# zhangyi-3/UCDIR

Hardware: AMD Instinct MI355X
Metric: restored images/sec at 50-step p_sample_loop, 256x256 SID (higher is better)
Workload: dtype bf16

## Files before the change

ucdir_amd/csrc/engine.hip:

```cpp
#include <hip/hip_runtime.h>

#include <cmath>
#include <cstdio>
#include <cstring>
#include <map>
#include <mutex>
#include <set>
#include <array>
#include <atomic>
#include <memory>
#include <string>
#include <vector>

#include "../../include/ucdir_hip.h"
#include "cgemm.hip.h"
#include "conv_halo.hip.h"
#include "akgm_halo.hip.h"
#include "akgm_pre.hip.h"
#include "akgm_ws.hip.h"
#include "akgm_ws32.hip.h"
#include "akgm_ws64.hip.h"
#include "conv_ws.hip.h"
#include "conv_sk.hip.h"
#include "conv_ws128.hip.h"
#include "flash_attn2.hip.h"
#include "qkv_ws.hip.h"
#include "common.h"
#include "misc.hip.h"
#include "fewstep.hip.h"
#include "image_metrics.hip.h"
#include "jpeg_roundtrip.hip.h"
#include "pack.h"

static thread_local std::string g_err;
static int fail(const std::string& m) { g_err = m; return 1; }
#define HIPC(x)                                                                                   \
    do {                                                                                          \
        hipError_t e_ = (x);                                                                      \
        if (e_ != hipSuccess) {                                                                   \
            throw std::runtime_error(std::string(#x) + ": " + hipGetErrorString(e_));             \
        }                                                                                         \
    } while (0)
#define API_BEGIN try {
#define API_END                                                                                   \
    }                                                                                             \
    catch (const std::exception& e) { return fail(e.what()); }                                    \
    catch (...) { return fail("unknown error"); }                                                 \
// ... 27 lines not shown
        return p;
    }
    static constexpr size_t STAT_CAP = 1 << 21;
    stat_t* stat_slab = nullptr; size_t stat_used = 0;
    stat_t* alloc_stats(int B) {
        if (!stat_slab) stat_slab = (stat_t*)alloc(STAT_CAP * sizeof(stat_t), true);
        const size_t n = (size_t)2 * UCDIR_STAT_SLOTS * B;
        if (stat_used + n > STAT_CAP) throw std::runtime_error("DevPool: statistics slab exhausted");
        stat_t* p = stat_slab + stat_used; stat_used += n;
        return p;
    }
    void zero_stats(hipStream_t st) { if (stat_used) HIPC(hipMemsetAsync(stat_slab, 0, stat_used * sizeof(stat_t), st)); }
    void release() { for (void* p : ptrs) (void)hipFree(p); ptrs.clear(); bytes = 0; stat_slab = nullptr; stat_used = 0; }
    ~DevPool() { release(); }
};

struct ConvW {
    bf16_t* A = nullptr; float* bias = nullptr; float* Tb = nullptr; float* Tg = nullptr;
    int rows_pad = 0, Kpad = 0, ntaps = 0, cin = 0, cout = 0, TM = 128; bool fold = false;
    bf16_t* Aup = nullptr; int Kup = 0;
    bf16_t* A10 = nullptr; float* bias_res = nullptr;
    bf16_t* Aws = nullptr;
    bf16_t* Aws128 = nullptr;
    bf16_t* Aqkv = nullptr;
    bf16_t* Atile = nullptr;
    bf16_t* Ask[2] = {nullptr, nullptr}; bf16_t* Ask_up[2] = {nullptr, nullptr};
    long long sk_up_stride[2] = {0, 0};
    bf16_t* Ask1x1 = nullptr;
};
struct AkgmW {
    bf16_t* A = nullptr; float* bias = nullptr; float* Tb = nullptr; float* Tg = nullptr;
    float* Tbb = nullptr;
    bf16_t* Apre = nullptr;
    bf16_t* Aws32 = nullptr;
    bf16_t* Aws64 = nullptr;
    int C = 0, cg = 0, Kpad = 0;
};

static int pick_tm(int cout) { return cout >= 128 ? 128 : 64; }

static ConvW upload_conv(DevPool& pool, const float* w, const float* bias, const float* gamma, const float* beta,
                         int cout, int cin, int ks) {
    ConvW W;
    W.TM = pick_tm(cout);
    PackedConv P = pack_conv(w, bias, gamma, beta, cout, cin, ks, W.TM);
    W.A = pool.upload(P.A); W.bias = pool.upload(P.bias);
// ... 103 lines not shown
    StampDump(hipStream_t, StampLayout) {}
    unsigned long long* dbg() const { return nullptr; }
    template <typename H> void print(H) const {}
#endif
};

struct Env {
    static bool has(const char* n) { return getenv(n) != nullptr; }
    static bool is0(const char* n) { const char* v = getenv(n); return v && atoi(v) == 0; }
    const bool no_pre = has("UCDIR_NO_PRE");
    const bool no_attlds = has("UCDIR_NO_ATTLDS");
    const bool no_ws = has("UCDIR_NO_WS");
    const bool no_ws16 = has("UCDIR_NO_WS16");
    const bool no_ws32 = has("UCDIR_NO_WS32");
    const bool no_ws64 = has("UCDIR_NO_WS64");
    const bool no_owntc = has("UCDIR_NO_OWNTC");
    const bool no_conv_sk = has("UCDIR_NO_CONV_SK");
    const bool sk_mix = !is0("UCDIR_SK_MIX");
    const bool no_tail_res = has("UCDIR_NO_TAIL_RES");
    const bool no_fused_res = has("UCDIR_NO_FUSED_RES");
    const bool no_atile = has("UCDIR_NO_ATILE");
    const bool no_conv_ws = has("UCDIR_NO_CONV_WS");
    const bool no_conv_ws128 = has("UCDIR_NO_CONV_WS128");
    const bool no_qkv_ws = has("UCDIR_NO_QKV_WS");
    const bool no_flash = has("UCDIR_NO_FLASH");
    const bool no_fused_final = has("UCDIR_NO_FUSED_FINAL");
    const bool splitk = !is0("UCDIR_SPLITK");
    const int splitk_wgs = has("UCDIR_SPLITK_WGS") ? atoi(getenv("UCDIR_SPLITK_WGS")) : 256;
    const bool keep_acts = has("UCDIR_KEEP_ACTS");
    const bool prof_detail = has("UCDIR_PROF_DETAIL");
};
static const Env& env() { static const Env e; return e; }

template <int TM, int EPI, int MODE>
static void launch_one(const GemmP& p, dim3 grid, size_t lds, hipStream_t st) {
    hipLaunchKernelGGL((cgemm_kernel<TM, EPI, MODE>), grid, dim3(CG_THREADS), lds, st, p);
}

template <typename K> static void set_lds_attr(K* k, int bytes, bool abs0 = false) {
    HIPC(hipFuncSetAttribute((const void*)k, hipFuncAttributeMaxDynamicSharedMemorySize, bytes));
    if (abs0) {
        hipFuncAttributes fa;
        HIPC(hipFuncGetAttributes(&fa, (const void*)k));
        require(fa.sharedSizeBytes == 0, "a kernel with absolute LDS addressing has static __shared__ memory: its dynamic smem[] no longer starts at offset 0");
    }
}
// ... 5 lines not shown
#define SPLITK_MAX_WGS 512
#define SK_MAX_GRID 256
#define SCRATCH_BYTES ((size_t)2 * SK_MAX_GRID * 65536 * sizeof(float))
static std::map<int, float*> g_splitk_buf;
static std::mutex g_static_mu;
static void ensure_kernel_attrs() {
    std::lock_guard<std::mutex> lk(g_static_mu);
    static std::set<int> done;
    int dev = 0;
    HIPC(hipGetDevice(&dev));
    if (done.count(dev)) return;
    set_cgemm_attrs<64>(); set_cgemm_attrs<128>();
    set_lds_attr(conv3x3_halo_kernel<128, false>, hc_lds_bytes<128>());
    set_lds_attr(conv3x3_halo_kernel<64, false>, hc_lds_bytes<64>());
    set_lds_attr(conv3x3_halo_kernel<64, true>, hc_lds_bytes<64>());
    set_lds_attr(akgm_halo_stage_kernel, AH_LDS); set_lds_attr(akgm_halo_kernel<true>, AH_LDS);
    set_lds_attr(akgm_pre_kernel<8>, AkPre<8>::LDS);
    set_lds_attr(akgm_ws_kernel<8>, AkWs::LDS); set_lds_attr(akgm_ws_kernel<16>, AkWs::LDS);
    set_lds_attr(akgm_ws32_kernel<32>, AkWs32::LDS); set_lds_attr(akgm_ws32_kernel<16>, AkWs32::LDS); set_lds_attr(akgm_ws32_kernel<8>, AkWs32::LDS);
    set_lds_attr(akgm_ws64_kernel<2, 8, true>, 160 * 1024); set_lds_attr(akgm_ws64_kernel<4, 8, true>, 160 * 1024);
    set_lds_attr(qkv_ws_kernel<256>, QkvWs::LDS); set_lds_attr(qkv_ws_kernel<512>, QkvWs::LDS);
    set_lds_attr(conv_ws_kernel, CvWs::LDS);
    set_lds_attr(conv_ws128_kernel, CvWs128::LDS);
    set_lds_attr(conv_sk_kernel<2, 8, 9>, 160 * 1024); set_lds_attr(conv_sk_kernel<2, 8, 4>, 160 * 1024);
    set_lds_attr(conv_sk_kernel<1, 8, 9>, 160 * 1024); set_lds_attr(conv_sk_kernel<1, 8, 4>, 160 * 1024);
    set_lds_attr(conv_sk_kernel<1, 4, 9>, 80 * 1024, true); set_lds_attr(conv_sk_kernel<1, 4, 4>, 80 * 1024, true);

    set_lds_attr(final_conv_kernel, 160 * 1024);
    set_lds_attr(flash_attn2_kernel<1, false>, fa_lds_bytes(128), true); set_lds_attr(flash_attn2_kernel<1, true>, fa_lds_bytes(128), true);
    set_lds_attr(flash_attn2_kernel<2, false>, fa_lds_bytes(256), true); set_lds_attr(flash_attn2_kernel<2, true>, fa_lds_bytes(256), true);
    set_lds_attr(flash_attn2_kernel<3, false>, fa_lds_bytes(384), true); set_lds_attr(flash_attn2_kernel<3, true>, fa_lds_bytes(384), true);
    set_lds_attr(flash_attn2_kernel<4, false>, fa_lds_bytes(512), true); set_lds_attr(flash_attn2_kernel<4, true>, fa_lds_bytes(512), true);
    done.insert(dev);
}

static void gemm_work(const GemmP& p, int epi, double& flops, double& bytes) {
    const double cols = ((p.cols_mode == COLS_PLAIN) ? (double)p.W : (double)p.H * p.W) * (p.up_phase ? 4.0 : 1.0);
    if (epi == EPI_AKGM) {
        const double C = 8.0 * p.cg;
        flops = 2.0 * 9 * C * C * cols * p.nbatch;
        bytes = (2.0 * C * cols * 2 + C * cols * 2 + cols * 32) * p.nbatch + 9.0 * C * C * 2;
    } else {
        const double K = (double)p.ntaps * p.cg;
        flops = 2.0 * K * p.nfeat * cols * p.nbatch;
        double in_cols = cols;
        if (p.cols_mode == COLS_DOWN) in_cols = cols * 4; else if (p.cols_mode == COLS_UP) in_cols = cols / 4;
// ... 66 lines not shown
    memo[{H, W}] = {th, tw};
}

template <int TM, bool DUAL = false>
static void launch_halo(GemmP p, hipStream_t st) {
    const int ks = p.ksplit > 1 ? p.ksplit : 1;
    const int nblk = p.nbatch * p.tiles_x * p.tiles_y * p.rowtiles * (p.up_phase ? 4 : 1) * ks + p.alt_blocks;
    ProfEntry e = gemm_entry((TM == 128 ? KEY_HALO128 : KEY_HALO64) + (p.up_phase ? KEY_HALO_UP : 0) + (DUAL ? KEY_HALO_DUAL : 0), p, EPI_STD, p.cg);
    if (p.alt_blocks) add_res_rider(e, p);
    StampDump sd(st, STAMPS_256); p.dbg = sd.dbg();
    bracket(e, st, [&] {
        hipLaunchKernelGGL((conv3x3_halo_kernel<TM, DUAL>), dim3(nblk), dim3(HC_THREADS), hc_lds_bytes<TM>(), st, p);
        if (ks == 1) return;
        const long long items = (long long)p.H * p.W * (p.up_phase ? 4 : 1) * (p.nfeat / 8);
        int gx = (int)((items + 255) / 256); if (gx > 1024) gx = 1024;
        hipLaunchKernelGGL(conv_splitk_finish_kernel, dim3(gx, p.nbatch), dim3(256), 0, st, p, TM);
    });
    sd.print([](int, int n) { fprintf(stderr, "TIMING n=%d:", n); });
}

static std::atomic<bool> g_use_halo{true};

static std::atomic<int> g_wsb{-1};
static std::atomic<int> g_persist_grid{0};
static int num_cus() {
    if (g_persist_grid > 0) return g_persist_grid;
    static std::map<int, int> memo;
    static std::mutex mu;
    std::lock_guard<std::mutex> lk(mu);
    int dev = 0;
    HIPC(hipGetDevice(&dev));
    auto it = memo.find(dev);
    if (it != memo.end()) return it->second;
    int n = 0;
    HIPC(hipDeviceGetAttribute(&n, hipDeviceAttributeMultiprocessorCount, dev));
    if (n <= 0) n = 256;
    memo[dev] = n;
    return n;
}

static thread_local float* t_splitk = nullptr;
static float* splitk_scratch() {
    if (t_splitk) return t_splitk;
    std::lock_guard<std::mutex> lk(g_static_mu);
    int dev = 0;
    HIPC(hipGetDevice(&dev));
// ... 148 lines not shown
                2.0 * 9 * cin * (double)w.cout * cols,
                ((double)cin * H * W * 2 + (double)w.cout * cols / B * 2) * B + 9.0 * cin * w.cout * 2, H, W, cin, w.cout};
    if (p.alt_units) { e.flops += 2.0 * cin * (double)w.cout * cols; e.bytes += 2.0 * cin * w.cout + 2.0 * w.cout * cols; }
    StampDump sd(st, STAMPS_CONV_SK); p.dbg = sd.dbg();
    bracket(e, st, [&] {
        if (upph) hipLaunchKernelGGL((conv_sk_kernel<MW, NW, 4>), dim3(G), dim3(L::THREADS), lds, st, p);
        else hipLaunchKernelGGL((conv_sk_kernel<MW, NW, 9>), dim3(G), dim3(L::THREADS), lds, st, p);
        if (nsk > 0) hipLaunchKernelGGL((conv_sk_finish_kernel<MW, NW>), dim3(4 * NW, nsk), dim3(64), 0, st, p, Gmain);
    });
    sd.print([&](int win, int n) { fprintf(stderr, "CONV_SK TIMING %s units=%d grid=%d n=%d:", win ? "last-round" : "first-round", p.units, G, n); });
    return true;
}
static bool try_conv_sk(const ConvW& w, ConvCall& c, bool upph, hipStream_t st) {
    const int mode = g_convsk.load();
    if (mode == 0 || (mode < 0 && env().no_conv_sk)) return false;
    if (c.x0.C % 32 || (c.x1 && c.x1->C % 32) || c.y.C % 8) return false;
    const int kind = mode > 0 ? mode : 2;
    const int fm = mode > 0 ? 1 : -1;
    if (kind == 2) return try_conv_sk_mw<1, 4>(w, c, upph, st, fm);
    if (w.cout % 256 == 0) return try_conv_sk_mw<2, 8>(w, c, upph, st, fm);
    return try_conv_sk_mw<1, 8>(w, c, upph, st, fm);
}

enum class ConvKind { WS128, WS, HALO128, HALO64, HALO64_DUAL, CGEMM };

static bool run_conv(const ConvW& w, int mode, ConvCall c, hipStream_t st) {
    const Act &x0 = c.x0, &y = c.y; const Act* x1 = c.x1;
    GemmP p; zero_gemm(p);
    const int cin = x0.C + (x1 ? x1->C : 0);
    require(cin == w.cin, "run_conv: channel mismatch");
    require(y.C == w.cout, "run_conv: cout mismatch");
    p.A = w.A; p.a_ld = w.Kpad; p.a_rows = w.rows_pad;
    p.B0 = x0.p; p.b0_bstride = x0.bstride(); p.ld0 = x0.C; p.c0 = x0.C;
    if (x1) { p.B1 = x1->p; p.b1_bstride = x1->bstride(); p.ld1 = x1->C; }
    p.cols_mode = mode;
    p.H = y.H; p.W = y.W; p.Wp = y.W + 2;
    p.Hi = x0.H; p.Wi = x0.W; p.Wpi = x0.W + 2;
    p.p0 = p.Wp + 1; p.pn = (y.H - 1) * p.Wp + y.W;
    p.ntaps = w.ntaps; p.cg = cin; p.cpt = cin / 8; p.cpt_shift = 0;
    p.nk = w.Kpad / CG_BK;
    p.tiles = (p.pn + CG_TP - 1) / CG_TP;
    p.rowtiles = w.rows_pad / w.TM;
    p.nbatch = y.B;
    p.fold = w.fold ? 1 : 0; p.act = c.act;
    if (w.fold) {
        p.stats0 = x0.stats; p.stats1 = x1 ? x1->stats : nullptr;
        p.inv_count = 1.0 / ((double)cin * x0.H * x0.W);
// ... 30 lines not shown
        p.A = w.A10; p.a_ld = 10 * cin; p.res_fused = 1; p.bias2 = w.bias_res;
        p.out2 = c.res_out->p; p.out2_bstride = c.res_out->bstride(); p.out2_ld = c.res_out->C;
        did_res = true;
    }
    const bool dual = did_res;
    if (!env().no_atile && halo && !upph && !did_res && tm_run == w.TM && w.Atile && w.ntaps == 9) p.A_tiled = w.Atile;
    if (halo && !did_res && !p.out_nchw && w.cout % 8 == 0) {
        const int taps = upph ? 4 : 9, tps = 256 / tm_run;
        const int ks = choose_ksplit(p.nbatch * p.tiles * p.rowtiles, cin / HC_BK, (taps + tps - 1) / tps,
                                     (double)y.B * y.H * y.W * w.cout);
        if (ks > 1) { p.ksplit = ks; p.partial = splitk_scratch(); }
    }
    if (halo && !upph && !did_res && c.res_out && c.wres && !env().no_tail_res && !p.out_nchw && c.wres->ntaps == 1 &&
        c.wres->rows_pad >= p.rowtiles * tm_run) {
        p.alt_blocks = p.nbatch * p.tiles * p.rowtiles;
        p.alt_A = c.wres->A; p.alt_a_ld = c.wres->Kpad; p.bias2 = c.wres->bias;
        p.out2 = c.res_out->p; p.out2_bstride = c.res_out->bstride(); p.out2_ld = c.res_out->C;
        did_res = true;
    }
    ConvKind kind = !halo ? ConvKind::CGEMM : tm_run == 128 ? ConvKind::HALO128 : dual ? ConvKind::HALO64_DUAL : ConvKind::HALO64;
    if (!env().no_conv_ws128 && dual && w.Aws128 && cin == 128 && x0.C == 64 && x1 && x1->C == 64 && !c.res && !p.out_nchw && y.H % 8 == 0 && y.W % 16 == 0 &&
        y.C == 64 && (g_persist_grid > 0 || (long long)y.B * (y.H / 8) * (y.W / 16) >= 4LL * num_cus()))
        kind = ConvKind::WS128;
    else if (!env().no_conv_ws && halo && !upph && !did_res && w.Aws && !x1 && !c.res && !p.out_nchw && p.ksplit <= 1 && !p.alt_blocks &&
             y.H % 16 == 0 && y.W % 16 == 0 && x0.C == 64 && y.C == 64 &&
             (g_persist_grid > 0 || (long long)y.B * (y.H / 16) * (y.W / 16) >= 4LL * num_cus()))
        kind = ConvKind::WS;

    switch (kind) {
        case ConvKind::WS128: {
            p.A = w.Aws128; p.alt_A = w.Aws128 + (size_t)2 * 72 * 2 * 32 * 8;
            p.th = 8; p.tw = 16; p.tiles_x = y.W / 16; p.tiles_y = y.H / 8;
            const int ntiles = y.B * p.tiles_x * p.tiles_y, ncu = num_cus();
            const int grid = ntiles < ncu ? ntiles : ncu;
            ProfEntry e = gemm_entry(KEY_CONV_WS128, p, EPI_STD, p.cg);
            add_res_rider(e, p);
            StampDump sd(st, STAMPS_256); p.dbg = sd.dbg();
            bracket(e, st, [&] { hipLaunchKernelGGL(conv_ws128_kernel, dim3(grid), dim3(CvWs128::THREADS), CvWs128::LDS, st, p); });
            sd.print([](int, int n) { fprintf(stderr, "CONV_WS128 TIMING n=%d:", n); });
            break;
        }
        case ConvKind::WS: {
            p.A = w.Aws; p.th = 16; p.tw = 16; p.tiles_x = y.W / 16; p.tiles_y = y.H / 16;
            const int ntiles = y.B * p.tiles_x * p.tiles_y, ncu = num_cus();
            const int grid = ntiles < ncu ? ntiles : ncu;
            StampDump sd(st, STAMPS_CONV_WS); p.dbg = sd.dbg();
            bracket(gemm_entry(KEY_CONV_WS, p, EPI_STD, p.cg), st, [&] { hipLaunchKernelGGL(conv_ws_kernel, dim3(grid), dim3(HC_THREADS), CvWs::LDS, st, p); });
            sd.print([](int win, int n) { fprintf(stderr, "CONV_WS TIMING %s n=%d:", win ? "late" : "early", n); });
            break;
        }
        case ConvKind::HALO128: launch_halo<128>(p, st); break;
        case ConvKind::HALO64_DUAL: launch_halo<64, true>(p, st); break;
        case ConvKind::HALO64: launch_halo<64>(p, st); break;
        case ConvKind::CGEMM: launch_cgemm(p, w.TM, EPI_STD, st); break;
    }
    return did_res;
}

enum class AkgmKind { WS64_4, WS64_2, WS32, WS, WS16, PRE, HALO_ATTLDS, HALO_STAGE };

static void run_akgm_halo(const AkgmW& w, const Act& h1, const float* G, const float* attw, const Act& res, Act& y, float* tcbuf, hipStream_t st) {
    const bool pre = !env().no_pre && w.Apre != nullptr && w.cg == 8;
// ... 427 lines not shown
            w.stem_w = c->wpool.upload(pack_stem_frags(t, W_(c, d.name + ".bias", (size_t)d.cout), 6, d.cout));
        } else if (d.kind == "down" || d.kind == "up") {
            w.conv = upload_conv(c->wpool, W_(c, d.name + ".conv.weight", (size_t)d.cout * d.cin * 9).data(),
                                 W_(c, d.name + ".conv.bias", d.cout).data(), nullptr, nullptr, d.cout, d.cin, 3);
            if (d.kind == "up") upload_upconv(c->wpool, w.conv, W_(c, d.name + ".conv.weight", (size_t)d.cout * d.cin * 9).data(),
                                              W_(c, d.name + ".conv.bias", d.cout).data());
        } else {
            const std::string r = d.name + ".res_block.";
            w.block_index = nb++;
            w.conv = upload_conv(c->wpool, W_(c, r + "conv1.weight", (size_t)d.cout * d.cin * 9).data(),
                                 W_(c, r + "conv1.bias", d.cout).data(), W_(c, r + "norm1.weight", d.cin).data(),
                                 W_(c, r + "norm1.bias", d.cin).data(), d.cout, d.cin, 3);
            w.has_res = d.cin != d.cout;
            if (w.has_res) {
                w.resconv = upload_conv(c->wpool, W_(c, r + "res_conv.weight", (size_t)d.cout * d.cin).data(),
                                        W_(c, r + "res_conv.bias", d.cout).data(), nullptr, nullptr, d.cout, d.cin, 1);
                if (w.conv.TM == 64 && d.cin % 64 == 0 && w.conv.Kpad == 9 * d.cin) {
                    PackedConv P = pack_conv(W_(c, r + "conv1.weight", (size_t)d.cout * d.cin * 9).data(), nullptr,
                                             W_(c, r + "norm1.weight", d.cin).data(), W_(c, r + "norm1.bias", d.cin).data(),
                                             d.cout, d.cin, 3, 64);
                    const std::vector<bf16_t> a10 = pack_conv_res10(P, W_(c, r + "res_conv.weight", (size_t)d.cout * d.cin).data());
                    w.conv.A10 = c->wpool.upload(a10);
                    if (d.cin == 128 && d.cout == 64) w.conv.Aws128 = c->wpool.upload(pack_conv_ws128(a10));
                    w.conv.bias_res = w.resconv.bias;
                }
            }
            w.sp = upload_akgm(c->wpool, W_(c, r + "spdyconv.weight", (size_t)8 * d.cout * (d.cout / 8) * 9).data(),
                               W_(c, r + "spdyconv.bias", (size_t)8 * d.cout).data(), W_(c, r + "norm2.weight", d.cout).data(),
                               W_(c, r + "norm2.bias", d.cout).data(), d.cout);
            std::vector<float> gw;
            for (const char* s : {"conv2.0.weight", "conv2.0.bias", "conv2.2.weight", "conv2.2.bias"}) {
                const auto& v = c->host.at(r + s).v;
                gw.insert(gw.end(), v.begin(), v.end());
            }
            require(gw.size() == 48 + 16 + 576 + 8, "guide branch weights have wrong size");
            w.gw = c->wpool.upload(gw);
            for (const char* s : {"noise_func.0.weight", "noise_func.0.bias", "noise_func.2.weight", "noise_func.2.bias"}) {
                const auto& v = c->host.at(r + s).v;
                tw.insert(tw.end(), v.begin(), v.end());
            }
            if (d.attn) {
                const std::string a = d.name + ".attn.";
                const std::vector<float> wf = fold_out_into_v(W_(c, a + "qkv.weight", (size_t)3 * d.cout * d.cout).data(),
                                                              W_(c, a + "out.weight", (size_t)d.cout * d.cout).data(), d.cout);
                w.qkv = upload_conv(c->wpool, wf.data(), nullptr,
                                    W_(c, a + "norm.weight", d.cout).data(), W_(c, a + "norm.bias", d.cout).data(),
// ... 557 lines not shown
        const Act* a = &r.out;
        if (!strcmp(what, "h1")) a = &r.h1;
        else if (!strcmp(what, "res")) a = &r.res;
        else if (!strcmp(what, "bo")) a = &r.bo;
        require(a->p != nullptr, "no such activation");
        const int64_t n = (int64_t)a->B * a->C * a->H * a->W;
        require(n == dst_elems, "debug_read: dst has " + std::to_string(dst_elems) + " elements, activation has " + std::to_string(n));
        hipLaunchKernelGGL(act_to_nchw_kernel, dim3(2048), dim3(256), 0, (hipStream_t)stream, a->p, dst, a->B, a->C, a->H, a->W);
        HIPC(hipGetLastError());
        return 0;
    }
    throw std::runtime_error(std::string("unknown layer ") + layer);
    API_END
}

int32_t ucdir_debug_flag(const char* name, int32_t value) {
    API_BEGIN
    require(name != nullptr, "null argument");
    if (!strcmp(name, "flash")) g_flash = value;
    else if (!strcmp(name, "splitk")) g_splitk = value;
    else if (!strcmp(name, "wsb")) g_wsb = value;
    else if (!strcmp(name, "skmix")) g_skmix = value;
    else if (!strcmp(name, "convsk")) g_convsk = value;
    else if (!strcmp(name, "persist_grid")) g_persist_grid = value;
    else throw std::runtime_error(std::string("unknown debug flag ") + name);
    API_END
}

int32_t ucdir_debug_launch_plan(const char* what, int32_t wgs, int32_t nchunks, int32_t steps_per_chunk, double out_elems) {
    if (!what) return -1;
    try {
        if (!strcmp(what, "ksplit")) return choose_ksplit(wgs, nchunks, steps_per_chunk, out_elems);
        if (!strcmp(what, "usplit")) return choose_usplit(wgs);
    } catch (...) {}
    return -1;
}

int32_t ucdir_profile_enable(int32_t on) {
    API_BEGIN
    g_prof.on = on != 0;
    API_END
}

int32_t ucdir_profile_read(int32_t cap, int32_t* keys, int32_t* launches, double* ms, double* flops, double* bytes,
                           int32_t* nrows, void* stream) {
    API_BEGIN
    HIPC(hipStreamSynchronize((hipStream_t)stream));
    std::map<int, int> idx; int n = 0;
    const bool detail = env().prof_detail;
    struct Det { int n = 0; double ms = 0, flops = 0; };
    std::map<std::array<int, 5>, Det> det;
    for (auto& e : g_prof.entries) {
        float t = 0.f; HIPC(hipEventElapsedTime(&t, e.e0, e.e1));
        if (detail) { Det& d = det[{e.key, e.dH, e.dW, e.dCin, e.dCout}]; d.n++; d.ms += t; d.flops += e.flops; }
        auto it = idx.find(e.key);
        int r;
// ... 78 lines not shown
    read_stats(out, B, stats_out_host, st);
    API_END
}

int32_t ucdir_op_conv_res(const float* x0, int32_t c0, const float* x1, int32_t c1, int32_t B, int32_t H, int32_t W,
                          const float* w_host, const float* bias_host, const float* gamma_host, const float* beta_host,
                          const float* wres_host, const float* bres_host, int32_t cout, int32_t silu,
                          float* y, float* yres, double* stats_out_host, void* stream) {
    API_BEGIN
    ensure_kernel_attrs();
    hipStream_t st = (hipStream_t)stream;
    DevPool pool;
    const int cin = c0 + (x1 ? c1 : 0);
    Act a0 = act_from_nchw(pool, x0, B, c0, H, W, st, true);
    Act a1; if (x1) a1 = act_from_nchw(pool, x1, B, c1, H, W, st, true);
    Act out = make_act(pool, B, H, W, cout), rout = make_act(pool, B, H, W, cout, false);
    ConvW w = upload_conv(pool, w_host, bias_host, gamma_host, beta_host, cout, cin, 3);
    ConvW wr = upload_conv(pool, wres_host, bres_host, nullptr, nullptr, cout, cin, 1);
    if (w.TM == 64 && cin % 64 == 0 && w.Kpad == 9 * cin) {
        PackedConv P = pack_conv(w_host, nullptr, gamma_host, beta_host, cout, cin, 3, 64);
        const std::vector<bf16_t> a10 = pack_conv_res10(P, wres_host);
        w.A10 = pool.upload(a10); w.bias_res = wr.bias;
        if (cin == 128 && cout == 64) w.Aws128 = pool.upload(pack_conv_ws128(a10));
    }
    const bool did = run_conv(w, COLS_S1, {a0, x1 ? &a1 : nullptr, out, silu, nullptr, true, &rout, &wr}, st);
    if (!did) run_conv(wr, COLS_S1, {a0, x1 ? &a1 : nullptr, rout, 0, nullptr, false}, st);
    hipLaunchKernelGGL(act_to_nchw_kernel, dim3(2048), dim3(256), 0, st, out.p, y, B, cout, H, W);
    hipLaunchKernelGGL(act_to_nchw_kernel, dim3(2048), dim3(256), 0, st, rout.p, yres, B, cout, H, W);
    HIPC(hipGetLastError());
    read_stats(out, B, stats_out_host, st);
    API_END
}

int32_t ucdir_op_akgm(const float* h, const float* att, const float* res, int32_t B, int32_t C, int32_t H, int32_t W,
                      const float* wsp_host, const float* bsp_host, const float* gamma_host, const float* beta_host,
                      float* y, double* stats_out_host, void* stream) {
    API_BEGIN
    ensure_kernel_attrs();
    hipStream_t st = (hipStream_t)stream;
    DevPool pool;
    Act ah = act_from_nchw(pool, h, B, C, H, W, st, true);
    Act ar = act_from_nchw(pool, res, B, C, H, W, st, false);
    Act out = make_act(pool, B, H, W, C);
    float* G = (float*)pool.alloc((size_t)B * H * W * 8 * 4);
    hipLaunchKernelGGL(nchw8_to_compact_kernel, dim3(1024), dim3(256), 0, st, att, G, B, H, W);
    std::vector<float> ones((size_t)B * 8, 1.f);
// ... 277 lines not shown
```

ucdir_amd/csrc/pack.h:

```cpp
#pragma once
#include <cmath>
#include <cstdint>
#include <vector>

#include "common.h"

struct PackedConv {
    std::vector<bf16_t> A;
    std::vector<float> bias;
    std::vector<float> Tb, Tg;
    int rows_pad = 0, Kpad = 0, ntaps = 0, cin = 0, cout = 0, ncls = 0;
};

static inline bool tap_valid(int cls, int tap) {
    const int cy = cls / 3, cx = cls % 3, ky = tap / 3, kx = tap % 3;
    if (cy == 0 && ky == 0) return false;
    if (cy == 2 && ky == 2) return false;
    if (cx == 0 && kx == 0) return false;
    if (cx == 2 && kx == 2) return false;
    return true;
}

static inline PackedConv pack_conv(const float* w, const float* bias, const float* gamma, const float* beta,
                                   int cout, int cin, int ks, int TM) {
// ... 43 lines not shown
        for (int j = 0; j < 36; ++j)
            for (int hk = 0; hk < 2; ++hk)
                for (int rho = 0; rho < 32; ++rho) {
                    const int o = 32 * rw + 16 * ((rho >> 2) & 1) + (rho & 3) + 4 * (rho >> 3);
                    const int tap = j >> 2, c0 = 16 * (j & 3) + 8 * hk;
                    for (int e = 0; e < 8; ++e)
                        img[((((size_t)rw * 36 + j) * 2 + hk) * 32 + rho) * 8 + e] = P.A[(size_t)o * P.Kpad + (size_t)tap * 64 + c0 + e];
                }
    return img;
}

static inline std::vector<bf16_t> pack_conv_ws128(const std::vector<bf16_t>& A10) {
    const int K10 = 10 * 128, nj = 80;
    std::vector<bf16_t> img((size_t)2 * nj * 2 * 32 * 8, 0);
    for (int rw = 0; rw < 2; ++rw)
        for (int j = 0; j < nj; ++j)
            for (int hk = 0; hk < 2; ++hk)
                for (int rho = 0; rho < 32; ++rho) {
                    const int o = 32 * rw + 16 * ((rho >> 2) & 1) + (rho & 3) + 4 * (rho >> 3);
                    const int tap = j >> 3, c0 = 16 * (j & 7) + 8 * hk;
                    const size_t dst = j < 72 ? ((((size_t)rw * 72 + j) * 2 + hk) * 32 + rho) * 8
                                              : (size_t)2 * 72 * 2 * 32 * 8 + ((((size_t)rw * 8 + (j - 72)) * 2 + hk) * 32 + rho) * 8;
                    for (int e = 0; e < 8; ++e) img[dst + e] = A10[(size_t)o * K10 + (size_t)tap * 128 + c0 + e];
                }
    return img;
}

static inline std::vector<bf16_t> pack_conv_res10(const PackedConv& P, const float* wres) {
    const int cin = P.cin, K10 = 10 * cin;
    std::vector<bf16_t> A((size_t)P.rows_pad * K10, 0);
    for (int o = 0; o < P.rows_pad; ++o) {
        for (int k = 0; k < 9 * cin; ++k) A[(size_t)o * K10 + k] = P.A[(size_t)o * P.Kpad + k];
        if (o < P.cout)
            for (int c = 0; c < cin; ++c) A[(size_t)o * K10 + 9 * cin + c] = f2bf(wres[(size_t)o * cin + c]);
    }
    return A;
}

struct PackedAkgm {
    std::vector<bf16_t> A;
    std::vector<float> bias;
    std::vector<float> Tb, Tg;
    int C = 0, cg = 0, Kpad = 0;
};

static inline PackedAkgm pack_akgm(const float* wsp, const float* bsp, const float* gamma, const float* beta, int C,
// ... 209 lines not shown
```

Before: 37.05.

## Add weight-stationary split-K conv kernel for 192-to-64 dual-input resblock convs

Adds a persistent weight-stationary 3x3 conv kernel for the 192-input (128+64 concatenated) to 64-output resblock conv with a fused 1x1 residual projection. Each of eight waves keeps its slice of the K dimension in registers and computes a partial sum. The partials are reduced through LDS, and the next halo tile is prefetched by DMA into a double buffer. The goal is to stop these layers falling back to the generic halo/cgemm path, which reloads weights on every tile. In exchange the kernel adds cross-wave reduction traffic and barriers, and it only runs when there are enough tiles to fill the persistent grid.

Result: no change. 37.13, median of 2 (+0.2%).

```diff
diff --git a/ucdir_amd/csrc/conv_wsq.hip.h b/ucdir_amd/csrc/conv_wsq.hip.h
--- /dev/null
+++ b/ucdir_amd/csrc/conv_wsq.hip.h
@@ -0,0 +1,349 @@
+#pragma once
+#include <type_traits>
+#include "conv_ws128.hip.h"
+
+struct CvWsq {
+    static constexpr int PITCH = 24;
+    static constexpr int PLANE = 6 * PITCH * 128;
+    static constexpr int HALO = 3 * PLANE;
+    static constexpr int NPIECE = HALO / 1024;
+    static constexpr int QSTEP = 2 * PITCH * 128;
+    static constexpr int SLOT = 16 * 32 * 4;
+    static constexpr int STAGE = 2 * 4 * 3 * SLOT;
+    static constexpr int OFF_STAGE2 = 2 * HALO;
+    static constexpr int OFF_TCS = OFF_STAGE2 + STAGE;
+    static constexpr int OFF_B2 = OFF_TCS + 9 * 64 * 4;
+    static constexpr int OFF_SCAL = OFF_B2 + 64 * 4;
+    static constexpr int LDS = OFF_SCAL + 128;
+    static constexpr int THREADS = 512;
+    static constexpr int NFRAG = 30;
+    static constexpr int A_WAVE = NFRAG * 2 * 32 * 8;
+};
+static_assert(CvWsq::LDS <= 160 * 1024, "conv_wsq: LDS budget");
+static_assert(CvWsq::STAGE <= CvWsq::HALO, "conv_wsq: the conv's stage must fit the halo buffer it aliases");
+
+__global__ __launch_bounds__(CvWsq::THREADS, 2) void conv_wsq_kernel(const GemmP p) {
+    using L = CvWsq;
+    extern __shared__ __attribute__((aligned(16))) unsigned char smem[];
+    float* const tcs = reinterpret_cast<float*>(smem + L::OFF_TCS);
+    float* const b2s = reinterpret_cast<float*>(smem + L::OFF_B2);
+    float* const scal = reinterpret_cast<float*>(smem + L::OFF_SCAL);
+    const int tid = threadIdx.x, lane = tid & 63, l31 = lane & 31, hh = lane >> 5;
+    const int wave = __builtin_amdgcn_readfirstlane(tid >> 6);
+    const int rw = wave & 1, q = wave >> 1;
+    const int prow = l31 >> 4; int pcol = (l31 & 15) ^ (prow << 3);
+    int lid;
+    {
+        const int nblk = gridDim.x, bid = blockIdx.x;
+        const int qq = nblk >> 3, r = nblk & 7, xcd = bid & 7;
+        lid = (xcd < r ? xcd * (qq + 1) : r * (qq + 1) + (xcd - r) * qq) + (bid >> 3);
+    }
+#ifdef UCDIR_TIMING
+    const bool dbg_on = p.dbg && (lid == (int)gridDim.x / 2 + 3) && (lane == 0) && (wave == 1);
+    int dbg_n = 0;
+#define CQ_STAMP() do { if (dbg_on && dbg_n < 250) p.dbg[dbg_n++] = __builtin_amdgcn_s_memtime(); } while (0)
+#else
+#define CQ_STAMP() do {} while (0)
+#endif
+    CQ_STAMP();
+    const int tps = p.tiles_x * p.tiles_y;
+    const int T = p.nbatch * tps;
+    const int t_beg = (int)((long long)lid * T / (int)gridDim.x), t_end = (int)((long long)(lid + 1) * T / (int)gridDim.x);
+    if (t_beg >= t_end) return;
+
+    bf16x8_t af[27], af2[3];
+    {
+        const bf16_t* Ab = p.A + (long long)wave * L::A_WAVE + (hh * 32 + l31) * 8;
+#pragma unroll
+        for (int j = 0; j < 27; ++j) af[j] = *reinterpret_cast<const bf16x8_t*>(Ab + j * (2 * 32 * 8));
+#pragma unroll
+        for (int j = 0; j < 3; ++j) af2[j] = *reinterpret_cast<const bf16x8_t*>(Ab + (27 + j) * (2 * 32 * 8));
+    }
+#pragma unroll
+    for (int j = 0; j < 27; ++j) asm volatile("" : "+v"(af[j]));
+#pragma unroll
+    for (int j = 0; j < 3; ++j) asm volatile("" : "+v"(af2[j]));
+    if (tid < 64) b2s[tid] = p.bias2 ? p.bias2[tid] : 0.f;
+
+    int l8 = lane >> 3;
+    unsigned hl0 = (unsigned)(l8 * p.ld0 * 2 + (((lane & 7) ^ (l8 >> 1)) << 4));
+    unsigned hl1 = (unsigned)(l8 * p.ld1 * 2 + (((lane & 7) ^ (l8 >> 1)) << 4));
+    unsigned ba[3][3];
+    {
+        const int hp0 = prow * L::PITCH + pcol;
+#pragma unroll
+        for (int s = 0; s < 3; ++s) {
+            const int ch0 = 48 * q + 16 * s, pl = ch0 >> 6, c16 = (ch0 & 63) >> 4;
+#pragma unroll
+            for (int kx = 0; kx < 3; ++kx) {
+                const int sxh = (((hp0 + kx) >> 1) & 7) ^ hh;
+                ba[s][kx] = pl * L::PLANE + ((hp0 + kx) << 7) + (((2 * c16) ^ sxh) << 4);
+            }
+        }
+    }
+    const unsigned st_lane = (unsigned)(((l31 & 15) * 2 + hh) * 16);
+    unsigned st_wr[2];
+#pragma unroll
+    for (int tp = 0; tp < 2; ++tp) {
+        const int d = 2 * tp + prow;
+        st_wr[tp] = (unsigned)(((rw * 4 + d) * 3 + (q - (q > d ? 1 : 0))) * L::SLOT) + st_lane;
+    }
+    unsigned st_rd = (unsigned)((rw * 4 + q) * 3 * L::SLOT) + st_lane;
+    const bool mine = prow == (q & 1);
+    unsigned tc_lane = L::OFF_TCS + (32 * rw + 16 * hh) * 4;
+    unsigned b2_lane = L::OFF_B2 + (32 * rw + 16 * hh) * 4;
+    unsigned rel_out = (unsigned)(((q + 1) * p.Wp + pcol + 1) * 64 + 32 * rw + 16 * hh) * 2;
+
+    int b, ty, tx;
+    {
+        b = t_beg / tps;
+        const int r = t_beg - b * tps;
+        ty = r / p.tiles_x; tx = r - ty * p.tiles_x;
+    }
+    auto issue_tile = [&](int nb, int nty, int ntx, int buf) {
+        const long long pix0 = (long long)nty * 4 * p.Wp + ntx * 16;
+        const unsigned char* h0 = reinterpret_cast<const unsigned char*>(p.B0 + (long long)nb * p.b0_bstride + pix0 * p.ld0);
+        const unsigned char* h1 = reinterpret_cast<const unsigned char*>(p.B1 + (long long)nb * p.b1_bstride + pix0 * p.ld1);
+        const int rv = p.H + 2 - nty * 4;
+        int cv = p.W + 2 - ntx * 16; cv = cv < 18 ? cv : 18;
+#pragma unroll
+        for (int i = 0; i < 7; ++i) {
+            const int e = wave + 8 * i;
+            if (e < L::NPIECE) {
+                const int pl = e / 18, r = (e - 18 * pl) / 3, c3 = e - 18 * pl - 3 * r;
+                const long long uoff = pl < 2 ? (long long)((r * p.Wp + c3 * 8) * p.ld0 + 64 * pl) * 2 : (long long)((r * p.Wp + c3 * 8) * p.ld1) * 2;
+                const unsigned long long sb = reinterpret_cast<unsigned long long>((pl < 2 ? h0 : h1) + uoff);
+                const unsigned long long sbu = ((unsigned long long)(unsigned)__builtin_amdgcn_readfirstlane((int)(sb >> 32)) << 32) | (unsigned)__builtin_amdgcn_readfirstlane((int)sb);
+                if (r < rv && c3 * 8 + l8 < cv)
+                    dma16_sbase(reinterpret_cast<const void*>(sbu), (pl < 2 ? hl0 : hl1) ^ (((r + c3) & 1) ? 64u : 0u), (unsigned)__builtin_amdgcn_readfirstlane(buf * L::HALO + e * 1024));
+            }
+        }
+    };
+    issue_tile(b, ty, tx, 0);
+
+    int b_cur = -1;
+    float rstd_a = 1.f;
+    stat_t S1 = 0, S2 = 0;
+    const int act = p.act;
+    const f32x16_t zero = {0.f, 0.f, 0.f, 0.f, 0.f, 0.f, 0.f, 0.f, 0.f, 0.f, 0.f, 0.f, 0.f, 0.f, 0.f, 0.f};
+
+#pragma unroll 1
+    for (int t = t_beg; t < t_end; ++t) {
+        const int buf = (t - t_beg) & 1;
+        const bool last = t + 1 == t_end;
+        asm volatile("" : "+v"(hl0), "+v"(hl1), "+v"(l8), "+v"(pcol), "+v"(tc_lane), "+v"(b2_lane), "+v"(rel_out), "+v"(st_rd), "+v"(st_wr[0]), "+v"(st_wr[1]));
+        CQ_STAMP();
+        if (t == t_beg) { HC_WAIT(0); }
+        asm volatile("s_barrier" ::: "memory");
+        CQ_STAMP();
+        if (b != b_cur) {
+            if (b_cur >= 0 && p.stats_out) {
+                const stat_t a = wave_sum_ll(S1), q2 = wave_sum_ll(S2);
+                if (lane == 0) stat_add_fx(p.stats_out, b_cur, a, q2);
+            }
+            S1 = 0; S2 = 0;
+            b_cur = b;
+            if (wave == 0) {
+                float mean = 0.f, rstd = 1.f;
+                if (p.fold) {
+                    long long v = 0;
+                    if (lane < 2 * UCDIR_STAT_SLOTS) {
+                        v = p.stats0[(long long)b * (2 * UCDIR_STAT_SLOTS) + lane];
+                        if (p.stats1) v += p.stats1[(long long)b * (2 * UCDIR_STAT_SLOTS) + lane];
+                    }
+#pragma unroll
+                    for (int off = 2; off < 2 * UCDIR_STAT_SLOTS; off <<= 1) v += __shfl_xor(v, off);
+                    const long long q2 = __shfl(v, 1);
+                    mean_rstd(stat_val(v), stat_val(q2), p.inv_count, mean, rstd);
+                }
+                if (lane == 0) { scal[0] = mean; scal[1] = rstd; }
+            }
+            __syncthreads();
+            const float mean = scal[0], rstd = scal[1];
+            for (int i = tid; i < 9 * 64; i += L::THREADS) {
+                const int cls = i >> 6, f = i & 63;
+                float v = p.bias ? p.bias[f] : 0.f;
+                if (p.fold) v += p.Tb[(long long)cls * p.tab_ld + f] - mean * rstd * p.Tg[(long long)cls * p.tab_ld + f];
+                tcs[i] = v;
+            }
+            rstd_a = __builtin_bit_cast(float, __builtin_amdgcn_readfirstlane(__builtin_bit_cast(int, p.alpha * (p.fold ? rstd : 1.0f))));
+            __syncthreads();
+        }
+        int nb = b, nty = ty, ntx = tx + 1;
+        if (ntx == p.tiles_x) { ntx = 0; if (++nty == p.tiles_y) { nty = 0; ++nb; } }
+        if (!last) issue_tile(nb, nty, ntx, buf ^ 1);
+        CQ_STAMP();
+
+        if (t != t_beg) {
+            const int d = buf ? L::HALO : -L::HALO;
+#pragma unroll
+            for (int s = 0; s < 3; ++s)
+#pragma unroll
+                for (int kx = 0; kx < 3; ++kx) ba[s][kx] += d;
+        }
+
+        f32x16_t acc[2];
+        {
+            bf16x8_t bq[3][2];
+            auto read_b = [&](auto jc, bf16x8_t (&dst)[2]) {
+                constexpr int j = decltype(jc)::value;
+                constexpr int tap = j / 3, s = j - 3 * tap, ky = tap / 3, kx = tap - 3 * ky;
+                const unsigned a = ky == 1 ? ba[s][kx] ^ 64u : ba[s][kx];
+                lds_read16_asm<ky * (L::PITCH * 128)>(dst[0], a);
+                lds_read16_asm<ky * (L::PITCH * 128) + L::QSTEP>(dst[1], a);
+            };
+            __builtin_amdgcn_sched_barrier(0);
+            asm volatile("s_waitcnt lgkmcnt(0)" ::: "memory");
+            read_b(std::integral_constant<int, 0>{}, bq[0]);
+            read_b(std::integral_constant<int, 1>{}, bq[1]);
+            __builtin_amdgcn_s_setprio(1);
+            static_for<0, 27>([&](auto jc) {
+                constexpr int j = decltype(jc)::value;
+                if constexpr (j + 2 < 27) read_b(std::integral_constant<int, j + 2>{}, bq[(j + 2) % 3]);
+                constexpr int younger = (j + 2 < 27) ? 4 : ((j + 1 < 27) ? 2 : 0);
+                lgkm_wait_asm<younger>();
+                acc[0] = __builtin_amdgcn_mfma_f32_32x32x16_bf16(af[j], bq[j % 3][0], j ? acc[0] : zero, 0, 0, 0);
+                acc[1] = __builtin_amdgcn_mfma_f32_32x32x16_bf16(af[j], bq[j % 3][1], j ? acc[1] : zero, 0, 0, 0);
+            });
+            __builtin_amdgcn_sched_barrier(0);
+            __builtin_amdgcn_s_setprio(0);
+        }
+        CQ_STAMP();
+        f32x16_t acc2[2];
+        {
+            bf16x8_t br[3][2];
+            __builtin_amdgcn_sched_barrier(0);
+            static_for<0, 3>([&](auto sc) {
+                constexpr int s = decltype(sc)::value;
+                lds_read16_asm<L::PITCH * 128>(br[s][0], ba[s][1] ^ 64u);
+                lds_read16_asm<L::PITCH * 128 + L::QSTEP>(br[s][1], ba[s][1] ^ 64u);
+            });
+            static_for<0, 3>([&](auto sc) {
+                constexpr int s = decltype(sc)::value;
+                lgkm_wait_asm<2 * (2 - s)>();
+                acc2[0] = __builtin_amdgcn_mfma_f32_32x32x16_bf16(af2[s], br[s][0], s ? acc2[0] : zero, 0, 0, 0);
+                acc2[1] = __builtin_amdgcn_mfma_f32_32x32x16_bf16(af2[s], br[s][1], s ? acc2[1] : zero, 0, 0, 0);
+            });
+            __builtin_amdgcn_sched_barrier(0);
+        }
+        CQ_STAMP();
+        asm volatile("s_barrier" ::: "memory");
+        CQ_STAMP();
+        float v[16], w[16];
+        {
+            unsigned char* const stc = smem + buf * L::HALO;
+#pragma unroll
+            for (int tp = 0; tp < 2; ++tp)
+                if (2 * tp + prow != q) {
+#pragma unroll
+                    for (int g4 = 0; g4 < 4; ++g4) {
+                        const f32x4_t v4 = {acc[tp][4 * g4], acc[tp][4 * g4 + 1], acc[tp][4 * g4 + 2], acc[tp][4 * g4 + 3]};
+                        *reinterpret_cast<f32x4_t*>(stc + st_wr[tp] + 512 * g4) = v4;
+                    }
+                }
+#pragma unroll
+            for (int i = 0; i < 16; ++i) v[i] = (q & 2) ? acc[1][i] : acc[0][i];
+            __builtin_amdgcn_sched_barrier(0);
+#pragma unroll
+            for (int tp = 0; tp < 2; ++tp)
+                if (2 * tp + prow != q) {
+#pragma unroll
+                    for (int g4 = 0; g4 < 4; ++g4) {
+                        const f32x4_t u4 = {acc2[tp][4 * g4], acc2[tp][4 * g4 + 1], acc2[tp][4 * g4 + 2], acc2[tp][4 * g4 + 3]};
+                        *reinterpret_cast<f32x4_t*>(smem + L::OFF_STAGE2 + st_wr[tp] + 512 * g4) = u4;
+                    }
+                }
+#pragma unroll
+            for (int i = 0; i < 16; ++i) w[i] = (q & 2) ? acc2[1][i] : acc2[0][i];
+        }
+        asm volatile("s_waitcnt lgkmcnt(0)\n\ts_barrier" ::: "memory");
+        CQ_STAMP();
+
+        auto finish = [&](auto qc) {
+            constexpr int Q = decltype(qc)::value;
+            const unsigned a_c = (unsigned)(buf * L::HALO) + st_rd, a_r = (unsigned)L::OFF_STAGE2 + st_rd;
+            f32x4_t ld[2][3];
+            auto rd = [&](auto kc, f32x4_t (&dst)[3]) {
+                constexpr int k = decltype(kc)::value;
+                const unsigned a = (k & 1) ? a_r : a_c;
+                lds_read16f_asm<512 * (k >> 1)>(dst[0], a);
+                lds_read16f_asm<512 * (k >> 1) + L::SLOT>(dst[1], a);
+                lds_read16f_asm<512 * (k >> 1) + 2 * L::SLOT>(dst[2], a);
+            };
+            __builtin_amdgcn_sched_barrier(0);
+            asm volatile("s_waitcnt lgkmcnt(0)" ::: "memory");
+            rd(std::integral_constant<int, 0>{}, ld[0]);
+            static_for<0, 8>([&](auto kc) {
+                constexpr int k = decltype(kc)::value, g4 = k >> 1;
+                if constexpr (k + 1 < 8) rd(std::integral_constant<int, k + 1>{}, ld[(k + 1) & 1]);
+                lgkm_wait_asm<(k + 1 < 8) ? 3 : 0>();
+#pragma unroll
+                for (int e = 0; e < 4; ++e) {
+                    const float o = (k & 1) ? w[4 * g4 + e] : v[4 * g4 + e];
+                    const float p0 = Q == 0 ? o : ld[k & 1][0][e];
+                    const float p1 = Q == 1 ? o : ld[k & 1][Q > 1 ? 1 : 0][e];
+                    const float p2 = Q == 2 ? o : ld[k & 1][Q > 2 ? 2 : 1][e];
+                    const float p3 = Q == 3 ? o : ld[k & 1][2][e];
+                    const float sum = ((p0 + p1) + p2) + p3;
+                    if constexpr (k & 1) w[4 * g4 + e] = sum; else v[4 * g4 + e] = sum;
+                }
+            });
+            __builtin_amdgcn_sched_barrier(0);
+        };
+        switch (q) {
+            case 0: finish(std::integral_constant<int, 0>{}); break;
+            case 1: finish(std::integral_constant<int, 1>{}); break;
+            case 2: finish(std::integral_constant<int, 2>{}); break;
+            default: finish(std::integral_constant<int, 3>{}); break;
+        }
+        const int gy = ty * 4 + q, gx = tx * 16 + pcol;
+        const bool valid = mine && gy < p.H && gx < p.W;
+        {
+            const int cy = gy == 0 ? 0 : (gy == p.H - 1 ? 2 : 1), cx = gx == 0 ? 0 : (gx == p.W - 1 ? 2 : 1);
+            const unsigned tca = tc_lane + (cy * 3 + cx) * 256;
+#pragma unroll
+            for (int g4 = 0; g4 < 4; ++g4) {
+                const f32x4_t c4 = *reinterpret_cast<const f32x4_t*>(smem + tca + 16 * g4);
+                const f32x4_t d4 = *reinterpret_cast<const f32x4_t*>(smem + b2_lane + 16 * g4);
+#pragma unroll
+                for (int e = 0; e < 4; ++e) {
+                    v[4 * g4 + e] = fmaf(v[4 * g4 + e], rstd_a, c4[e]);
+                    w[4 * g4 + e] = w[4 * g4 + e] + d4[e];
+                }
+            }
+        }
+        if (act == 1) {
+#pragma unroll
+            for (int i = 0; i < 16; ++i) v[i] = silu_fast(v[i]);
+        } else if (act == 2) {
+#pragma unroll
+            for (int i = 0; i < 16; ++i) v[i] = fmaxf(0.2f * v[i], v[i]);
+        }
+        float s1 = 0.f, s2 = 0.f;
+#pragma unroll
+        for (int i = 0; i < 16; ++i) { s1 += v[i]; s2 += v[i] * v[i]; }
+        if (!valid) { s1 = 0.f; s2 = 0.f; }
+        const uint4 pk0 = pack8_bf16(v), pk1 = pack8_bf16(v + 8), pk2 = pack8_bf16(w), pk3 = pack8_bf16(w + 8);
+        CQ_STAMP();
+        HC_WAIT(0);
+        CQ_STAMP();
+        if (valid) {
+            const long long tile_el = (long long)(ty * 4 * p.Wp + tx * 16) * 64;
+            unsigned char* outb = reinterpret_cast<unsigned char*>(reinterpret_cast<bf16_t*>(p.out) + (long long)b * p.out_bstride + tile_el) + rel_out;
+            unsigned char* out2b = reinterpret_cast<unsigned char*>(p.out2 + (long long)b * p.out2_bstride + tile_el) + rel_out;
+            *reinterpret_cast<uint4*>(outb) = pk0;
+            *reinterpret_cast<uint4*>(outb + 16) = pk1;
+            *reinterpret_cast<uint4*>(out2b) = pk2;
+            *reinterpret_cast<uint4*>(out2b + 16) = pk3;
+        }
+        S1 += stat_fx((double)s1); S2 += stat_fx((double)s2);
+        b = nb; ty = nty; tx = ntx;
+    }
+#ifdef UCDIR_TIMING
+    if (dbg_on) p.dbg[255] = dbg_n;
+#endif
+    if (p.stats_out) {
+        const stat_t a = wave_sum_ll(S1), q2 = wave_sum_ll(S2);
+        if (lane == 0) stat_add_fx(p.stats_out, b_cur, a, q2);
+    }
+}
diff --git a/ucdir_amd/csrc/engine.hip b/ucdir_amd/csrc/engine.hip
--- a/ucdir_amd/csrc/engine.hip
+++ b/ucdir_amd/csrc/engine.hip
@@ -23,6 +23,7 @@
 #include "conv_ws.hip.h"
 #include "conv_sk.hip.h"
 #include "conv_ws128.hip.h"
+#include "conv_wsq.hip.h"
 #include "flash_attn2.hip.h"
 #include "qkv_ws.hip.h"
 #include "common.h"
@@ -96,6 +97,7 @@
     bf16_t* A10 = nullptr; float* bias_res = nullptr;
     bf16_t* Aws = nullptr;
     bf16_t* Aws128 = nullptr;
+    bf16_t* Awsq = nullptr;
     bf16_t* Aqkv = nullptr;
     bf16_t* Atile = nullptr;
     bf16_t* Ask[2] = {nullptr, nullptr}; bf16_t* Ask_up[2] = {nullptr, nullptr};
@@ -245,6 +247,7 @@
     const bool no_atile = has("UCDIR_NO_ATILE");
     const bool no_conv_ws = has("UCDIR_NO_CONV_WS");
     const bool no_conv_ws128 = has("UCDIR_NO_CONV_WS128");
+    const bool no_conv_wsq = has("UCDIR_NO_CONV_WSQ");
     const bool no_qkv_ws = has("UCDIR_NO_QKV_WS");
     const bool no_flash = has("UCDIR_NO_FLASH");
     const bool no_fused_final = has("UCDIR_NO_FUSED_FINAL");
@@ -296,6 +299,7 @@
     set_lds_attr(qkv_ws_kernel<256>, QkvWs::LDS); set_lds_attr(qkv_ws_kernel<512>, QkvWs::LDS);
     set_lds_attr(conv_ws_kernel, CvWs::LDS);
     set_lds_attr(conv_ws128_kernel, CvWs128::LDS);
+    set_lds_attr(conv_wsq_kernel, CvWsq::LDS, true);
     set_lds_attr(conv_sk_kernel<2, 8, 9>, 160 * 1024); set_lds_attr(conv_sk_kernel<2, 8, 4>, 160 * 1024);
     set_lds_attr(conv_sk_kernel<1, 8, 9>, 160 * 1024); set_lds_attr(conv_sk_kernel<1, 8, 4>, 160 * 1024);
     set_lds_attr(conv_sk_kernel<1, 4, 9>, 80 * 1024, true); set_lds_attr(conv_sk_kernel<1, 4, 4>, 80 * 1024, true);
@@ -408,6 +412,7 @@
 static std::atomic<bool> g_use_halo{true};
 
 static std::atomic<int> g_wsb{-1};
+static std::atomic<int> g_wsq_launches{0};
 static std::atomic<int> g_persist_grid{0};
 static int num_cus() {
     if (g_persist_grid > 0) return g_persist_grid;
@@ -602,7 +607,7 @@
     return try_conv_sk_mw<1, 8>(w, c, upph, st, fm);
 }
 
-enum class ConvKind { WS128, WS, HALO128, HALO64, HALO64_DUAL, CGEMM };
+enum class ConvKind { WS128, WSQ, WS, HALO128, HALO64, HALO64_DUAL, CGEMM };
 
 static bool run_conv(const ConvW& w, int mode, ConvCall c, hipStream_t st) {
     const Act &x0 = c.x0, &y = c.y; const Act* x1 = c.x1;
@@ -679,6 +684,9 @@
     if (!env().no_conv_ws128 && dual && w.Aws128 && cin == 128 && x0.C == 64 && x1 && x1->C == 64 && !c.res && !p.out_nchw && y.H % 8 == 0 && y.W % 16 == 0 &&
         y.C == 64 && (g_persist_grid > 0 || (long long)y.B * (y.H / 8) * (y.W / 16) >= 4LL * num_cus()))
         kind = ConvKind::WS128;
+    else if (!env().no_conv_wsq && dual && w.Awsq && cin == 192 && x0.C == 128 && x1 && x1->C == 64 && !c.res && !p.out_nchw && y.C == 64 &&
+             (g_persist_grid > 0 || (long long)y.B * ((y.H + 3) / 4) * ((y.W + 15) / 16) >= 8LL * num_cus()))
+        kind = ConvKind::WSQ;
     else if (!env().no_conv_ws && halo && !upph && !did_res && w.Aws && !x1 && !c.res && !p.out_nchw && p.ksplit <= 1 && !p.alt_blocks &&
              y.H % 16 == 0 && y.W % 16 == 0 && x0.C == 64 && y.C == 64 &&
              (g_persist_grid > 0 || (long long)y.B * (y.H / 16) * (y.W / 16) >= 4LL * num_cus()))
@@ -695,6 +703,18 @@
             StampDump sd(st, STAMPS_256); p.dbg = sd.dbg();
             bracket(e, st, [&] { hipLaunchKernelGGL(conv_ws128_kernel, dim3(grid), dim3(CvWs128::THREADS), CvWs128::LDS, st, p); });
             sd.print([](int, int n) { fprintf(stderr, "CONV_WS128 TIMING n=%d:", n); });
+            break;
+        }
+        case ConvKind::WSQ: {
+            ProfEntry e = gemm_entry(KEY_HALO64 + KEY_HALO_DUAL, p, EPI_STD, p.cg);
+            p.A = w.Awsq;
+            p.th = 4; p.tw = 16; p.tiles_x = (y.W + 15) / 16; p.tiles_y = (y.H + 3) / 4;
+            const int ntiles = y.B * p.tiles_x * p.tiles_y, ncu = num_cus();
+            const int grid = ntiles < ncu ? ntiles : ncu;
+            StampDump sd(st, STAMPS_256); p.dbg = sd.dbg();
+            bracket(e, st, [&] { hipLaunchKernelGGL(conv_wsq_kernel, dim3(grid), dim3(CvWsq::THREADS), CvWsq::LDS, st, p); });
+            ++g_wsq_launches;
+            sd.print([](int, int n) { fprintf(stderr, "CONV_WSQ TIMING n=%d:", n); });
             break;
         }
         case ConvKind::WS: {
@@ -1168,6 +1188,7 @@
                     const std::vector<bf16_t> a10 = pack_conv_res10(P, W_(c, r + "res_conv.weight", (size_t)d.cout * d.cin).data());
                     w.conv.A10 = c->wpool.upload(a10);
                     if (d.cin == 128 && d.cout == 64) w.conv.Aws128 = c->wpool.upload(pack_conv_ws128(a10));
+                    if (d.cin == 192 && d.cout == 64) w.conv.Awsq = c->wpool.upload(pack_conv_wsq(a10));
                     w.conv.bias_res = w.resconv.bias;
                 }
             }
@@ -1771,6 +1792,7 @@
     else if (!strcmp(name, "wsb")) g_wsb = value;
     else if (!strcmp(name, "skmix")) g_skmix = value;
     else if (!strcmp(name, "convsk")) g_convsk = value;
+    else if (!strcmp(name, "conv_wsq_launches")) g_wsq_launches = value;
     else if (!strcmp(name, "persist_grid")) g_persist_grid = value;
     else throw std::runtime_error(std::string("unknown debug flag ") + name);
     API_END
@@ -1781,6 +1803,7 @@
     try {
         if (!strcmp(what, "ksplit")) return choose_ksplit(wgs, nchunks, steps_per_chunk, out_elems);
         if (!strcmp(what, "usplit")) return choose_usplit(wgs);
+        if (!strcmp(what, "conv_wsq_launches")) return g_wsq_launches.load();
     } catch (...) {}
     return -1;
 }
@@ -1905,6 +1928,7 @@
         const std::vector<bf16_t> a10 = pack_conv_res10(P, wres_host);
         w.A10 = pool.upload(a10); w.bias_res = wr.bias;
         if (cin == 128 && cout == 64) w.Aws128 = pool.upload(pack_conv_ws128(a10));
+        if (cin == 192 && cout == 64) w.Awsq = pool.upload(pack_conv_wsq(a10));
     }
     const bool did = run_conv(w, COLS_S1, {a0, x1 ? &a1 : nullptr, out, silu, nullptr, true, &rout, &wr}, st);
     if (!did) run_conv(wr, COLS_S1, {a0, x1 ? &a1 : nullptr, rout, 0, nullptr, false}, st);
diff --git a/ucdir_amd/csrc/pack.h b/ucdir_amd/csrc/pack.h
--- a/ucdir_amd/csrc/pack.h
+++ b/ucdir_amd/csrc/pack.h
@@ -89,6 +89,22 @@
                     const size_t dst = j < 72 ? ((((size_t)rw * 72 + j) * 2 + hk) * 32 + rho) * 8
                                               : (size_t)2 * 72 * 2 * 32 * 8 + ((((size_t)rw * 8 + (j - 72)) * 2 + hk) * 32 + rho) * 8;
                     for (int e = 0; e < 8; ++e) img[dst + e] = A10[(size_t)o * K10 + (size_t)tap * 128 + c0 + e];
+                }
+    return img;
+}
+
+static inline std::vector<bf16_t> pack_conv_wsq(const std::vector<bf16_t>& A10) {
+    const int K10 = 10 * 192, nj = 30;
+    std::vector<bf16_t> img((size_t)8 * nj * 2 * 32 * 8, 0);
+    for (int w = 0; w < 8; ++w)
+        for (int j = 0; j < nj; ++j)
+            for (int hk = 0; hk < 2; ++hk)
+                for (int rho = 0; rho < 32; ++rho) {
+                    const int rw = w & 1, q = w >> 1;
+                    const int o = 32 * rw + 16 * ((rho >> 2) & 1) + (rho & 3) + 4 * (rho >> 3);
+                    const int tap = j < 27 ? j / 3 : 9, s = j < 27 ? j % 3 : j - 27, c0 = 48 * q + 16 * s + 8 * hk;
+                    for (int e = 0; e < 8; ++e)
+                        img[((((size_t)w * nj + j) * 2 + hk) * 32 + rho) * 8 + e] = A10[(size_t)o * K10 + (size_t)tap * 192 + c0 + e];
                 }
     return img;
 }
```
